# jantonguirao/nvImageCodec

Hardware: AMD Instinct MI355X
Metric: images/sec, batched 1920x1080 4:2:0 baseline JPEG decode to interleaved RGB u8 (higher is better)
Workload: dtype int32

## Files before the change

include/hipjpeg.h:

```cpp
#ifndef HIPJPEG_H_
#define HIPJPEG_H_

#include <stddef.h>
#include <stdint.h>

#ifdef __cplusplus
extern "C" {
#endif

#define HIPJPEG_API __attribute__((visibility("default")))

typedef enum {
    HIPJPEG_STATUS_SUCCESS = 0,
    HIPJPEG_STATUS_INVALID_ARGUMENT = 1,
    HIPJPEG_STATUS_BAD_JPEG = 2,
    HIPJPEG_STATUS_UNSUPPORTED = 3,
    HIPJPEG_STATUS_TRUNCATED = 4,
    HIPJPEG_STATUS_CORRUPT = 5,
    HIPJPEG_STATUS_ALLOC_FAILED = 6,
    HIPJPEG_STATUS_HIP_ERROR = 7,
    HIPJPEG_STATUS_NO_DEVICE = 8,
    HIPJPEG_STATUS_BUFFER_TOO_SMALL = 9,
    HIPJPEG_STATUS_INTERNAL_ERROR = 10
} hipjpegStatus_t;
// ... 44 lines not shown
    int32_t x0, y0, x1, y1;
    int32_t orientation;
} hipjpegTransform_t;

typedef struct hipjpegHandle* hipjpegHandle_t;

HIPJPEG_API const char* hipjpegStatusString(hipjpegStatus_t status);
HIPJPEG_API int hipjpegVersion(void);
HIPJPEG_API hipjpegStatus_t hipjpegTestSetFault(const char* site, int countdown);
HIPJPEG_API int hipjpegTestDoubleReports(void);
HIPJPEG_API int32_t hipjpegTestHostFallbacks(hipjpegHandle_t handle);
HIPJPEG_API hipjpegStatus_t hipjpegTestKernelFlavours(hipjpegHandle_t handle, int32_t plane_units[1], int32_t luma_units[3]);
HIPJPEG_API int32_t hipjpegTestFusedUnits(hipjpegHandle_t handle);

HIPJPEG_API int32_t hipjpegTestScanChunkDrops(const uint8_t* data, size_t length, int scan_index, uint32_t* drops, int32_t capacity);

HIPJPEG_API hipjpegStatus_t hipjpegGetImageInfo(const uint8_t* data, size_t length, hipjpegImageInfo_t* info);

HIPJPEG_API hipjpegStatus_t hipjpegEntropyDecodeHost(const uint8_t* data, size_t length, int16_t* coef, size_t coef_capacity_bytes,
                                                     uint64_t comp_offsets[4], uint16_t qtables[256]);

HIPJPEG_API hipjpegStatus_t hipjpegEntropyDecodeHostSparse(const uint8_t* data, size_t length, uint8_t* stream, size_t capacity_bytes, size_t* stream_bytes,
                                                           uint64_t table_offsets[4]);

HIPJPEG_API hipjpegStatus_t hipjpegEntropyDecodeGpuAlgorithmHost(const uint8_t* data, size_t length, int16_t* coef,
                                                                 size_t coef_capacity_bytes, uint64_t comp_offsets[4],
                                                                 int32_t* sync_passes);

HIPJPEG_API hipjpegStatus_t hipjpegCreate(hipjpegHandle_t* handle, int device_id, int num_host_threads);
HIPJPEG_API hipjpegStatus_t hipjpegDestroy(hipjpegHandle_t handle);
// ... 133 lines not shown
```

nvimagecodec_amd/_native.py:

```python
import ctypes
import os
import sys

_HERE = os.path.dirname(os.path.abspath(__file__))
LIB_PATH = os.environ.get("HIPJPEG_LIB_PATH") or os.path.join(_HERE, "libhipjpeg_ext.so")

STATUS_NAMES = {0: "SUCCESS", 1: "INVALID_ARGUMENT", 2: "BAD_JPEG", 3: "UNSUPPORTED", 4: "TRUNCATED", 5: "CORRUPT", 6: "ALLOC_FAILED",
                7: "HIP_ERROR", 8: "NO_DEVICE", 9: "BUFFER_TOO_SMALL", 10: "INTERNAL_ERROR"}

OUTPUT_RGBI, OUTPUT_BGRI, OUTPUT_RGB_PLANAR, OUTPUT_BGR_PLANAR, OUTPUT_Y, OUTPUT_YUV_PLANAR = range(6)
FLAG_FANCY_UPSAMPLING = 1
FLAG_GPU_HUFFMAN = 2
FLAG_GPU_RESTART_INTERVALS = 8
TRANSCODE_ORIENTATION_FROM_EXIF = 0x10000
TRANSCODE_TRIM = 0x20000
TRANSCODE_GRAYSCALE = 0x80000
TRANSCODE_CROP_EXPAND = 0x100000
TRANSCODE_COPY_MARKERS = 0x200000
FLAG_FAST_IDCT = 4


class HipJpegError(RuntimeError):
    def __init__(self, status, what=""):
        self.status = int(status)
# ... 89 lines not shown
    L.hipjpegDecodeBatchStats.argtypes = [vp, vp, vp, vp]
    L.hipjpegDecodeBatchGetStatuses.argtypes = [vp, vp, i32]
    L.hipjpegDecodeBatchSetTransforms.argtypes = [vp, vp, i32]
    L.hipjpegDecodeBatchSubmit.argtypes = [vp, vp, vp, i32, vp, i32, ctypes.c_uint, vp]
    L.hipjpegDecodeBatchWait.argtypes = [vp, vp, i32]
    L.hipjpegSetPipelineDepth.argtypes = [vp, i32]
    L.hipjpegSetHybridHuffmanThreshold.argtypes = [vp, ctypes.c_uint64]
    L.hipjpegDecodeBatchTransferStats.argtypes = [vp, ctypes.POINTER(ctypes.c_uint64), ctypes.POINTER(ctypes.c_int32)]
    L.hipjpegEntropyDecodeHostSparse.argtypes = [vp, sz, vp, sz, ctypes.POINTER(sz), vp]
    L.hipjpegDecodeBatchZeroCopyImages.argtypes = [vp]
    L.hipjpegDecodeBatchZeroCopyImages.restype = i32
    L.hipjpegTestHostFallbacks.argtypes = [vp]
    L.hipjpegTestHostFallbacks.restype = i32
    L.hipjpegTestScanChunkDrops.argtypes = [vp, ctypes.c_size_t, i32, ctypes.POINTER(ctypes.c_uint32), i32]
    L.hipjpegTestScanChunkDrops.restype = i32
    L.hipjpegTestKernelFlavours.argtypes = [vp, ctypes.POINTER(ctypes.c_int32), ctypes.POINTER(ctypes.c_int32)]
    L.hipjpegDecodeBatchEntropyStats.argtypes = [vp, ctypes.POINTER(ctypes.c_int32), ctypes.POINTER(ctypes.c_int32), ctypes.POINTER(ctypes.c_uint64)]
    L.hipjpegEncodeBatchDevice.argtypes = [vp, vp, vp, i32, vp, vp]
    L.hipjpegEncodeBatchRelaunch.argtypes = [vp, vp]
    L.hipjpegEncodeBatchHost.argtypes = [vp, vp]
    L.hipjpegEncodeBatchEntropy.argtypes = [vp, ctypes.c_uint, vp]
    L.hipjpegEncodeBatchSubmit.argtypes = [vp, vp, vp, i32, ctypes.c_uint, vp]
    L.hipjpegEncodeBatchWait.argtypes = [vp, vp, i32]
    L.hipjpegEncodeBatch.argtypes = [vp, vp, vp, i32, vp, vp]
    L.hipjpegEncodeGetBitstream.argtypes = [vp, i32, ctypes.POINTER(vp), ctypes.POINTER(sz)]
    L.hipjpegEncodeGetCoefficients.argtypes = [vp, i32, i32, ctypes.POINTER(vp), vp]
    L.hipjpegEncodeBatchStats.argtypes = [vp, vp, vp, vp]
    L.hipjpegEncodeBatchGpuEntropyImages.argtypes = [vp]
    L.hipjpegEncodeBatchGpuEntropyImages.restype = i32
    L.hipjpegEncodeFromCoefficientsHost.argtypes = [i32, i32, ctypes.POINTER(EncodeParams), vp, vp, sz, ctypes.POINTER(sz)]
# ... 21 lines not shown
```

nvimagecodec_amd/csrc/gpu_huffman.hip:

```cpp
#include <hip/hip_runtime.h>

#include "gpu_huffman.h"
#include "huffman_gpu_core.h"

namespace hipjpeg {

namespace {

constexpr int kThreads = 256;

constexpr int kRowShift = kSubseqWords == 32 ? 5 : kSubseqWords == 16 ? 4 : kSubseqWords == 64 ? 6 : -1;
static_assert(kRowShift > 0, "subsequences of 512, 1024 or 2048 bits");

#define HJ_LDS __attribute__((address_space(3)))
#define HJ_GLOBAL __attribute__((address_space(1)))
typedef unsigned int u32x4 __attribute__((ext_vector_type(4)));

struct KSlot {
    int16_t* base;
    uint32_t stride_y, stride_x;
};

constexpr int kStagedExtra = 2;
constexpr int kRowWords = kSubseqWords + kStagedExtra;
// ... 9 lines not shown
};

__device__ __forceinline__ uint32_t load_boundary(const uint32_t* boundaries, uint32_t n, uint32_t i)
{
    return i < n ? ((const HJ_GLOBAL uint32_t*)boundaries)[i] : 0xFFFFFFFFu;
}
#ifndef HJ_WALK_PARTS
#define HJ_WALK_PARTS 15
#endif
constexpr int kWalkParts = HJ_WALK_PARTS;
static_assert((kWalkParts & 4) == 0 || (kWalkParts & 3) == 3, "the select form needs the registers and the long step");
constexpr bool kLaneRegisters = (kWalkParts & 9) == 1, kLaneLongStep = (kWalkParts & 10) == 2;
typedef WalkPolicy<(kWalkParts & 2) != 0, (kWalkParts & 4) != 0> SyncWalk;
typedef WalkPolicy<kLaneLongStep, false> LaneWalk;

template <bool IN_VGPRS>
__device__ __forceinline__ TableClasses table_classes(const HuffImage& im)
{
    TableClasses c = make_table_classes(im.blocks_per_mcu, [&](uint32_t q) { return ((uint32_t)im.k[q].tdc * 2) | ((uint32_t)im.k[q].tac * 2 << 16); });
#pragma unroll
    for (int i = 0; i < 4; i++) {
        c.pair[i] = HJ_UNIFORM(c.pair[i]);
        if (IN_VGPRS) asm("" : "+v"(c.pair[i]));
    }
    c.bit0 = HJ_UNIFORM(c.bit0);
    c.bit1 = HJ_UNIFORM(c.bit1);
    return c;
}

struct DevEnv {
    uint32_t stream_base;
    uint32_t word0;
    uint32_t row_addr;
    uint32_t row_word0;
    uint32_t pool;
    const HJ_LDS uint32_t* tsel;
    TableClasses classes;
    const uint32_t* boundaries;
    uint32_t num_boundaries;
    __device__ __forceinline__ uint32_t boundary(uint32_t i) const { return load_boundary(boundaries, num_boundaries, i); }
    static constexpr uint32_t kCursorStep = (uint32_t)kSyncThreads * 4u;
    __device__ __forceinline__ void set_row(int row)
    {
        row_addr = stream_base + ((uint32_t)row << 2);
        row_word0 = word0 + ((uint32_t)row << kRowShift);
    }
    __device__ __forceinline__ uint32_t cursor(uint32_t i) const { return row_addr + (i - row_word0) * kCursorStep; }
    __device__ __forceinline__ uint32_t fetch(uint32_t c) const { return *(const HJ_LDS uint32_t*)(uintptr_t)c; }
    __device__ __forceinline__ uint32_t tables(int k) const { return kLaneRegisters ? select_tables(classes, (uint32_t)k) : tsel[k]; }
    __device__ __forceinline__ uint32_t lookup1(uint32_t t, uint32_t w) const
    {
        return *(const HJ_LDS uint16_t*)(uintptr_t)(pool + t + ((w >> (31 - kHuffFastBits)) & ((2u << kHuffFastBits) - 2)));
// ... 31 lines not shown
    return r;
}
__device__ __forceinline__ void put_mark(const SlotRecorder& r, uint32_t begin, uint32_t limit, uint32_t total_bits, uint32_t z0, const SubseqState& st)
{
    *(HJ_GLOBAL uint16_t*)(r.records + (r.off + 2 * kRecMark)) = (uint16_t)record_mark(begin, min(limit, total_bits), z0, st);
}

template <class Policy, class Env>
__device__ __forceinline__ SubseqState walk_with(bool rst, bool record, const HuffGeom& geom, const Env& env, uint32_t begin, uint32_t limit, int z, int k,
                                                 uint32_t boundary0, const SlotRecorder& rec)
{
    if (rst) return decode_subsequence<true, Env, NoRecord, Policy>(geom, env, begin, limit, z, k, boundary0);
    return record ? decode_subsequence<false, Env, SlotRecorder, Policy>(geom, env, begin, limit, z, k, 0, rec)
                  : decode_subsequence<false, Env, NoRecord, Policy>(geom, env, begin, limit, z, k);
}
template <class Env>
struct FourClasses : Env {
    __device__ __forceinline__ explicit FourClasses(const Env& e) : Env(e) {}
    __device__ __forceinline__ uint32_t tables(int k) const { return select_tables(this->classes, (uint32_t)k); }
};
template <class Env>
struct TwoClasses : Env {
    __device__ __forceinline__ explicit TwoClasses(const Env& e) : Env(e) {}
    __device__ __forceinline__ uint32_t tables(int k) const { return select_tables2(this->classes, (uint32_t)k); }
};
template <class Policy, class Env>
__device__ __forceinline__ SubseqState walk_subsequence(bool rst, bool record, const HuffGeom& geom, const Env& env, uint32_t begin, uint32_t limit, int z,
                                                        int k, uint32_t boundary0, const SlotRecorder& rec)
{
    if (Policy::kSelects) {
        if (env.classes.bit1 == 0) return walk_with<Policy>(rst, record, geom, TwoClasses<Env>(env), begin, limit, z, k, boundary0, rec);
        return walk_with<Policy>(rst, record, geom, FourClasses<Env>(env), begin, limit, z, k, boundary0, rec);
    }
    return walk_with<Policy>(rst, record, geom, env, begin, limit, z, k, boundary0, rec);
}

template <int ROWS>
__device__ __forceinline__ void stage_rows(uint32_t* lds_stream, const HuffImage& im, int first_row)
{
    const int t = threadIdx.x;
    const HJ_GLOBAL uint32_t* g = (const HJ_GLOBAL uint32_t*)im.stream;
    const int nwords = (int)im.stream_words;
    const int w0 = (first_row + t) * kSubseqWords;
    constexpr int kGroups = kSubseqWords / 4;
    u32x4 v[kGroups];
    typedef unsigned int u32x2 __attribute__((ext_vector_type(2)));
    u32x2 tail;
    {
        const int gd = w0 + kSubseqWords;
// ... 53 lines not shown
        constexpr uint8_t zz[64] = HJ_ZIGZAG_DEVICE_TABLE;
        const int i = (t - 64) * 4;
        zzw[t - 64] = ((uint32_t)zz[i] | ((uint32_t)zz[i + 1] << 8) | ((uint32_t)zz[i + 2] << 16) | ((uint32_t)zz[i + 3] << 24)) << 1;
    }
}

__device__ __forceinline__ DevEnv make_env(WgShared& sh, HJ_LDS uint16_t* pool, uint32_t first, const HuffGeom& geom, const HuffImage& im)
{
    DevEnv env;
    env.stream_base = (uint32_t)(uintptr_t)(HJ_LDS uint32_t*)sh.stream;
    env.word0 = (first - 1) * kSubseqWords;
    env.row_addr = env.stream_base;
    env.row_word0 = env.word0;
    env.pool = (uint32_t)(uintptr_t)pool;
    env.tsel = (const HJ_LDS uint32_t*)sh.tsel;
    env.classes = table_classes<true>(im);
    env.boundaries = geom.boundaries;
    env.num_boundaries = geom.num_boundaries;
    return env;
}

__device__ __forceinline__ int compact_tasks(WgShared& sh, bool has, int value, int* task)
{
    const int t = threadIdx.x;
    const unsigned long long mask = __ballot(has);
    const int below = __popcll(mask & ((1ull << (t & 63)) - 1));
    if ((t & 63) == 0) sh.wave_count[t >> 6] = (uint32_t)__popcll(mask);
    __syncthreads();
    int base = 0, n = 0;
#pragma unroll
    for (int w = 0; w < kSyncThreads / 64; w++) {
// ... 1304 lines not shown
```

nvimagecodec_amd/csrc/gpu_huffman_host.cpp:

```cpp
#include "gpu_huffman_host.h"

#include <algorithm>
#include <cstring>

namespace hipjpeg {

uint32_t scan_mcus_x(const FrameInfo& f, const ScanHeader& sc)
{
    return (uint32_t)(sc.ncomp == 1 ? (f.comp[sc.comp_index[0]].samp_w + 7) / 8 : f.mcus_x);
}

uint32_t scan_mcus_y(const FrameInfo& f, const ScanHeader& sc)
{
    return (uint32_t)(sc.ncomp == 1 ? (f.comp[sc.comp_index[0]].samp_h + 7) / 8 : f.mcus_y);
}

uint32_t scan_blocks_per_mcu(const FrameInfo& f, const ScanHeader& sc)
{
    if (sc.ncomp == 1) return 1;
    uint32_t n = 0;
    for (int i = 0; i < sc.ncomp; i++) n += (uint32_t)(f.comp[sc.comp_index[i]].h * f.comp[sc.comp_index[i]].v);
    return n;
}

// ... 109 lines not shown
        } else {
            const uint32_t prefix = code >> (l - kHuffFastBits);
            if ((first[prefix] >> 9) != kZadvLong) {
                first[prefix] = (uint16_t)(((base + used) / 64) | (kZadvLong << 9));
                for (int j = 0; j < (1 << kHuffSubBits); j++) pool[base + used + j] = (uint16_t)kEntryInvalid;
                used += 1u << kHuffSubBits;
            }
            uint16_t* sub = pool + (size_t)(first[prefix] & 0x1FFu) * 64;
            const uint32_t lo = (code & ((1u << (l - kHuffFastBits)) - 1)) << (16 - l);
            for (uint32_t j = 0; j < (1u << (16 - l)); j++) sub[lo + j] = e;
        }
    });
    if (!is_dc) {
        uint16_t* pair = first + kPairOffset;
        for (uint32_t w = 0; w < (1u << kHuffFastBits); w++) {
            pair[w] = 0;
            const uint32_t e1 = first[w], t1 = e1 & 31u, z1 = e1 >> 9;
            if (e1 == kEntryInvalid || z1 == kZadvLong || z1 == 64u || t1 + 2 > (uint32_t)kHuffFastBits) continue;
            const uint32_t e2 = first[(w << t1) & ((1u << kHuffFastBits) - 1)], t2 = e2 & 31u, z2 = e2 >> 9;
            if (e2 == kEntryInvalid || z2 == kZadvLong || t1 + t2 > (uint32_t)kHuffFastBits) continue;
            pair[w] = (uint16_t)make_pair_entry(t1 + t2, z2 == 64u ? 63u : z1 + z2, 64u - z1);
        }
    }
    return used;
}

}

size_t gpu_pool_words(const ScanHeader& sc)
{
    size_t words = 0;
    bool dc_seen[4] = {false, false, false, false}, ac_seen[4] = {false, false, false, false};
    for (int i = 0; i < sc.ncomp; i++) {
        const int td = sc.td[i], ta = sc.ta[i];
        if (!dc_seen[td]) {
            dc_seen[td] = true;
// ... 26 lines not shown
    }
    for (int i = 0; i < sc.ncomp; i++) {
        const int ta = sc.ta[i];
        if (!ac_seen[ta]) {
            ac_seen[ta] = true;
            ac_off[ta] = used;
            used += expand_table(sc.ac[ta], false, pool, used);
        }
    }
    im->pool_words = (uint32_t)used;
    for (uint32_t k = 0; k < im->blocks_per_mcu; k++) {
        const int c = im->k[k].comp;
        im->k[k].tdc = (uint16_t)dc_off[sc.td[c]];
        im->k[k].tac = (uint16_t)ac_off[sc.ta[c]];
    }
}

void fill_huff_image(const FrameInfo& f, const ScanHeader& sc, uint32_t stream_bytes, HuffImage* im)
{
    memset(im, 0, sizeof *im);
    im->total_bits = stream_bytes * 8u;
    im->num_subseq = (im->total_bits + kSubseqBits - 1) / kSubseqBits;
    im->stream_words = (uint32_t)((((size_t)stream_bytes + 3) & ~(size_t)3) + kStreamSlackBytes) / 4;
    im->mcus_x = scan_mcus_x(f, sc);
    im->mcus_y = scan_mcus_y(f, sc);
    im->ncomp = (uint32_t)sc.ncomp;
    int k = 0;
    for (int i = 0; i < sc.ncomp; i++) {
        const Component& fc = f.comp[sc.comp_index[i]];
        const int h = sc.ncomp == 1 ? 1 : fc.h, v = sc.ncomp == 1 ? 1 : fc.v;
// ... 31 lines not shown
    uint32_t second_table(uint32_t e) const { return (e & 0x1FFu) * 64u; }
    uint32_t lookup_pair(uint32_t t, uint32_t w) const
    {
        const size_t i = (size_t)t + kPairOffset + (w >> (32 - kHuffFastBits));
        return i < im->pool_words ? im->pool[i] : 0u;
    }
    uint32_t tables(int k) const { return (uint32_t)im->k[k].tdc | ((uint32_t)im->k[k].tac << 16); }
    int16_t* block_ptr(int k, uint32_t mx, uint32_t my) const
    {
        const HuffK& hk = im->k[k];
        return im->coef[hk.comp] + ((size_t)hk.blk0 + (size_t)my * hk.stride_y + (size_t)mx * hk.stride_x) * 64;
    }
    int zigzag(int z) const { return kZigzagDeviceGpuHost[z]; }
    int16_t* buf;
    void put(int index, int value) const { buf[index] = (int16_t)value; }
};

struct HostWindow {
    const HostEnv* env;
    uint32_t edc[64], eac[64];
    uint32_t tables(uint32_t k) const { return env->tables((int)k); }
    uint32_t entry(uint32_t table, uint32_t w) const
    {
        uint32_t e = env->lookup1(table, w);
        if ((e >> 9) == kZadvLong) e = env->lookup2(e, w);
        return e;
    }
    void open(uint32_t pos, uint32_t ts)
    {
        for (uint32_t l = 0; l < 64; l++) {
// ... 34 lines not shown
    im.pool = pool.data();
    im.dc_diff = dc_diff.data();
    im.boundaries = boundaries.data();
    im.num_boundaries = (uint32_t)boundaries.size();
    im.restart_interval = (uint32_t)sc.restart_interval;
    const bool rst = sc.restart_interval != 0;
    for (int i = 0; i < sc.ncomp; i++) {
        const int c = sc.comp_index[i];
        int16_t* const coef = frame_coef[c];
        im.coef[i] = coef;
        const size_t bw = (size_t)f.comp[c].blocks_w, rows = sc.ncomp == 1 ? im.mcus_y : (size_t)f.comp[c].blocks_h;
        const size_t cols = sc.ncomp == 1 ? im.mcus_x : bw;
        for (size_t y = 0; y < rows; y++) memset(coef + y * bw * 64, 0x5A, cols * 128);
    }
    int16_t block_buffer[64] = {0};
    const HostEnv env{&im, block_buffer};
    const HuffGeom geom = make_geom(im);
    const uint32_t ns = im.num_subseq;
    std::vector<SubseqState> cur(ns), nxt(ns);
    uint32_t err = 0;
    std::vector<uint16_t> records((size_t)ns * kRecShorts, 0);
    {
        const TableClasses classes = make_table_classes(im.blocks_per_mcu, [&](uint32_t q) { return env.tables((int)q); });
        if (!classes.complete) return 5;
        for (uint32_t q = 0; q < im.blocks_per_mcu; q++)
            if (select_tables(classes, q) != env.tables((int)q)) return 5;
    }
    bool policies_differ = false;
    uint16_t other[kRecShorts];
    auto walk = [&](uint32_t i, uint32_t begin, int z, int k, bool record) {
        const uint32_t limit = (i + 1) * kSubseqBits;
        uint16_t* rec = &records[(size_t)i * kRecShorts];
        if (rst) {
            rec[kRecMark] = (uint16_t)kRecInvalid;
            const SubseqState st = decode_subsequence<true, HostEnv, NoRecord, WalkSelects>(geom, env, begin, limit, z, k, 0);
            if (pack_state(st) != pack_state(decode_subsequence<true, HostEnv, NoRecord, WalkBranches>(geom, env, begin, limit, z, k, 0)) ||
                pack_state(st) != pack_state(decode_subsequence<true, HostEnv, NoRecord, WalkLongBranches>(geom, env, begin, limit, z, k, 0)))
                policies_differ = true;
            return st;
        }
        if (!record) {
// ... 136 lines not shown
```

nvimagecodec_amd/csrc/gpu_huffman_host.h:

```cpp
#pragma once
#include <cstddef>
#include <cstdint>
#include <vector>

#include "huffman_gpu_core.h"
#include "jpeg_syntax.h"

namespace hipjpeg {

constexpr int kMaxSeqScans = 4;
bool gpu_entropy_eligible(const FrameInfo& f);

uint32_t scan_mcus_x(const FrameInfo& f, const ScanHeader& sc);
uint32_t scan_mcus_y(const FrameInfo& f, const ScanHeader& sc);
uint32_t scan_blocks_per_mcu(const FrameInfo& f, const ScanHeader& sc);

inline size_t destuffed_capacity(const ScanHeader& sc) { return (((sc.data_end - sc.data_begin) + 3) & ~(size_t)3) + kStreamSlackBytes; }

size_t destuff_scan(const uint8_t* data, const ScanHeader& sc, uint8_t* out);

size_t gpu_pool_words(const ScanHeader& sc);

void build_gpu_pool(const ScanHeader& sc, HuffImage* im, uint16_t* pool);

void fill_huff_image(const FrameInfo& f, const ScanHeader& sc, uint32_t stream_bytes, HuffImage* im);

int emulate_gpu_entropy(const uint8_t* data, size_t size, const FrameInfo& f, int16_t* const coef[4], int* sync_passes);

}
```

nvimagecodec_amd/csrc/hipjpeg_api.cpp:

```cpp
#include <hip/hip_runtime_api.h>

#include <cstring>
#include <memory>
#include <new>
#include <vector>

#include "../../include/hipjpeg.h"
#include "coefficients_core.h"
#include "decoder_core.h"
#include "diagnostics.h"
#include "encoder_core.h"
#include "entropy_decode.h"
#include "gpu_huffman_encode.h"
#include "gpu_huffman_host.h"
#include "progressive_encode.h"
#include "progressive_gpu_host.h"
#include "thread_pool.h"
#include "transcode_core.h"

#include <chrono>
#include <future>
#include <cstdio>
#include <cstdlib>

// ... 463 lines not shown
int32_t hipjpegTestScanChunkDrops(const uint8_t* data, size_t length, int scan_index, uint32_t* drops, int32_t capacity)
{
    int32_t result = -1;
    if (!test_hooks_enabled()) return result;
    (void)guarded([&]() -> hipjpegStatus_t {
        hipjpeg::FrameInfo f;
        if (hipjpeg::parse_jpeg(data, length, &f) != hipjpeg::kParseOk || scan_index < 0 || scan_index >= (int)f.scans.size()) return HIPJPEG_STATUS_BAD_JPEG;
        const auto& d = f.scans[scan_index].chunk_drops;
        for (int32_t c = 0; c < (int32_t)d.size() && c < capacity && drops; c++) drops[c] = d[c];
        result = (int32_t)d.size();
        return HIPJPEG_STATUS_SUCCESS;
    });
    return result;
}

int32_t hipjpegTestHostFallbacks(hipjpegHandle_t handle)
{
    if (!handle || !test_hooks_enabled()) return -1;
    return handle->batches[handle->settled >= 0 ? handle->settled : handle->current]->host_fallback_images();
}

hipjpegStatus_t hipjpegTestKernelFlavours(hipjpegHandle_t handle, int32_t plane_units[1], int32_t luma_units[3])
{
    return guarded([&]() -> hipjpegStatus_t {
    if (!handle || !plane_units || !luma_units || !test_hooks_enabled()) return HIPJPEG_STATUS_INVALID_ARGUMENT;
    handle->cur().flavour_units(plane_units, luma_units);
    return HIPJPEG_STATUS_SUCCESS;
    });
}

// ... 422 lines not shown
```

nvimagecodec_amd/csrc/huffman_gpu_core.h:

```cpp
#pragma once
#include <cstdint>
#include <type_traits>

#if defined(__HIPCC__)
#include <hip/hip_runtime.h>
#define HJ_HD __host__ __device__ inline __attribute__((always_inline))
#else
#define HJ_HD inline
#endif

namespace hipjpeg {

#ifndef HJ_SUBSEQ_BITS
#define HJ_SUBSEQ_BITS 1024
#endif
#ifndef HJ_SYNC_THREADS
#define HJ_SYNC_THREADS 256
#endif
constexpr int kSubseqBits = HJ_SUBSEQ_BITS;
constexpr int kSubseqWords = kSubseqBits / 32;
constexpr int kHuffFastBits = 10;
constexpr int kHuffSubBits = 16 - kHuffFastBits;
constexpr int kStreamSlackBytes = 32;
constexpr int kSyncThreads = HJ_SYNC_THREADS;
constexpr int kHuffOwn = kSyncThreads - 1;
constexpr int kTailTaskBytes = 2 * kSyncThreads;
constexpr int kHuffBlocksPerWg = 256;
#ifndef HJ_MCUS_PER_WG
#define HJ_MCUS_PER_WG 128
#endif
constexpr int kHuffMcusPerWg = HJ_MCUS_PER_WG;
constexpr int kDestuffChunk = 16384;
constexpr int kMaxPoolWords = 12288;

HJ_HD constexpr uint32_t make_entry(uint32_t total, uint32_t nb, uint32_t zadv) { return total | (nb << 5) | (zadv << 9); }
constexpr uint32_t kPairOffset = 1u << kHuffFastBits;
HJ_HD constexpr uint32_t make_pair_entry(uint32_t total, uint32_t zadv, uint32_t z_below) { return total | (zadv << 4) | (z_below << 10); }
constexpr uint32_t kEntryInvalid = 1u | (15u << 5) | (1u << 9);
constexpr uint32_t kZadvLong = 127;

struct HuffK {
    uint32_t blk0;
    uint32_t stride_y;
    uint16_t tdc, tac;
    uint8_t comp;
    uint8_t stride_x;
    uint8_t pad[2];
};

struct alignas(16) HuffImage {
    const uint8_t* stream;
    const uint16_t* pool;
    int16_t* coef[4];
    int16_t* dc_diff;
// ... 200 lines not shown
HJ_HD uint32_t bit_select(uint32_t mask, uint32_t ones, uint32_t zeros) { return (mask & ones) | (~mask & zeros); }
HJ_HD uint32_t bit_mask(uint32_t bits, uint32_t k)
{
#if defined(__HIP_DEVICE_COMPILE__)
    return (uint32_t)__builtin_amdgcn_sbfe((int)bits, k, 1u);
#else
    return 0u - ((bits >> k) & 1u);
#endif
}
HJ_HD uint32_t select_tables(const TableClasses& c, uint32_t k)
{
    const uint32_t a = bit_mask(c.bit0, k), b = bit_mask(c.bit1, k);
    return bit_select(b, bit_select(a, c.pair[3], c.pair[2]), bit_select(a, c.pair[1], c.pair[0]));
}
HJ_HD uint32_t select_tables2(const TableClasses& c, uint32_t k) { return bit_select(bit_mask(c.bit0, k), c.pair[1], c.pair[0]); }

template <bool LONG_STEP, bool SELECTS>
struct WalkPolicy {
    static constexpr bool kLongStep = LONG_STEP, kSelects = SELECTS;
    static_assert(LONG_STEP || !SELECTS, "the select form has no memory read to predicate");
};
typedef WalkPolicy<false, false> WalkBranches;
typedef WalkPolicy<true, false> WalkLongBranches;
typedef WalkPolicy<true, true> WalkSelects;
HJ_HD uint32_t sub_window(uint32_t w) { return (w << kHuffFastBits) >> (kHuffFastBits - kHuffSubBits); }

template <bool RST, class Env, class Rec = NoRecord, class Policy = WalkBranches>
HJ_HD SubseqState decode_subsequence(const HuffGeom& im, const Env& env, uint32_t begin, uint32_t limit, int z, int k, uint32_t boundary0 = 0,
                                     Rec rec = Rec())
{
    static_assert(!RST || std::is_same<Rec, NoRecord>::value, "records are not taken across restart boundaries");
    uint32_t pos = begin, nblocks = 0;
    const uint32_t end = limit < im.total_bits ? limit : im.total_bits;
    const uint32_t pair_end = end > (uint32_t)kHuffFastBits - 2 ? end - ((uint32_t)kHuffFastBits - 2) : 0;
    const int bpm = (int)im.blocks_per_mcu;
    uint32_t tsel = env.tables(k);
    uint32_t tcur = z == 0 ? (tsel & 0xFFFFu) : (tsel >> 16);
    BitReader br;
    br.start(env, pos);
    RestartCursor rc;
    if (RST) {
        rc.start(env, boundary0, pos);
        if (rc.normalise(env, br.hi, &pos, &z, &k)) {
            tsel = env.tables(k);
            tcur = tsel & 0xFFFFu;
            br.start(env, pos);
        }
    }
    const uint32_t fresh = z == 0 ? 1u : 0u;
    if (fresh && pos < end) rec(0u, pos);
    uint32_t win = br.hi;
    bool sub = false;
    while (pos < end) {
        const uint32_t fetched = env.fetch(br.next);
        uint32_t e = env.lookup1(tcur, win);
        const uint32_t pr = env.lookup_pair(tcur, win);
        const bool two = z != 0 && (uint32_t)z < (pr >> 10) && pos < pair_end && !sub;
        uint32_t tot = two ? (pr & 15u) : (e & 31u);
        bool mcu_done = false;
        if (Policy::kSelects) {
            const uint32_t zadv1 = e >> 9, zadv2 = (pr >> 4) & 63u, t2 = env.second_table(e);
            const bool lng = !two & (zadv1 == kZadvLong) & !sub;
            tot = lng ? 0u : tot;
            uint32_t zadv = two ? zadv2 : zadv1;
            zadv = lng ? 0u : zadv;
            z += (int)zadv;
            const bool done = z >= 64;
            if (done) rec(nblocks + fresh, pos + tot);
            z = done ? 0 : z;
            nblocks += done ? 1u : 0u;
            int k1 = k + 1;
            k1 = k1 == bpm ? 0 : k1;
            k = done ? k1 : k;
            tsel = env.tables(k);
            const uint32_t tdc = tsel & 0xFFFFu, tac = tsel >> 16;
            tcur = lng ? t2 : tac;
            tcur = done ? tdc : tcur;
            mcu_done = done & (k == 0);
            sub = lng;
        } else if (Policy::kLongStep) {
            const bool was_sub = sub;
            sub = false;
            tcur = tsel >> 16;
            z += two ? (int)((pr >> 4) & 63u) : (int)(e >> 9);
            if (z >= 64) {
                if (!two && (e >> 9) == kZadvLong && !was_sub) {
                    z -= (int)kZadvLong;
                    tot = 0;
                    tcur = env.second_table(e);
                    sub = true;
                } else {
                    z = 0;
                    rec(nblocks + fresh, pos + tot);
                    nblocks++;
                    if (++k == bpm) k = 0;
                    tsel = env.tables(k);
                    tcur = tsel & 0xFFFFu;
                    mcu_done = k == 0;
                }
            }
        } else {
            tcur = tsel >> 16;
            z += two ? (int)((pr >> 4) & 63u) : (int)(e >> 9);
            if (z >= 64) {
                if (!two && (e >> 9) == kZadvLong) {
                    e = env.lookup2(e, br.hi);
                    z += (int)(e >> 9) - (int)kZadvLong;
                    tot = e & 31u;
                }
                if (z >= 64) {
                    z = 0;
                    rec(nblocks + fresh, pos + tot);
                    nblocks++;
                    if (++k == bpm) k = 0;
                    tsel = env.tables(k);
                    tcur = tsel & 0xFFFFu;
                    mcu_done = k == 0;
                }
            }
        }
        pos += tot;
        br.consume(tot, fetched);
        if (RST && mcu_done && rc.normalise(env, br.hi, &pos, &z, &k)) {
            tsel = env.tables(k);
            tcur = tsel & 0xFFFFu;
            br.start(env, pos);
        }
        const uint32_t behind = sub_window(br.hi);
        win = sub ? behind : br.hi;
    }
    SubseqState st;
    st.end_bit = pos;
    st.zk = (uint16_t)((k << 8) | z);
    st.nblocks = (uint16_t)(nblocks > 0xFFFF ? 0xFFFF : nblocks);
    return st;
}

#if defined(__HIP_DEVICE_COMPILE__)
#define HJ_UNIFORM(x) ((uint32_t)__builtin_amdgcn_readfirstlane((int)(x)))
#else
#define HJ_UNIFORM(x) ((uint32_t)(x))
#endif
template <class Win>
HJ_HD uint32_t cooperative_table_changes(const Win& win, uint32_t blocks_per_mcu)
// ... 70 lines not shown
        rc.start(env, boundary0, pos);
        const uint32_t met = rc.index;
        if (rc.normalise(env, br.hi, &pos, &z, &k, fault)) {
            tsel = env.tables(k);
            tcur = tsel & 0xFFFFu;
            br.start(env, pos);
            fresh = true;
        }
        if (fault && rc.index != met && block != (met + 1) * im.interval_blocks) *fault = 1;
    }
    if (fresh && pos < end) rec(block, pos);
    while (pos < end) {
        const uint32_t fetched = env.fetch(br.next);
        uint32_t e = env.lookup1(tcur, br.hi);
        const uint32_t pr = env.lookup_pair(tcur, br.hi);
        const bool two = z != 0 && (uint32_t)z < (pr >> 10) && pos < pair_end;
        if (!two && (e >> 9) == kZadvLong) e = env.lookup2(e, br.hi);
        const uint32_t tot = two ? (pr & 15u) : (e & 31u);
        pos += tot;
        br.consume(tot, fetched);
        z += two ? (int)((pr >> 4) & 63u) : (int)(e >> 9);
        tcur = tsel >> 16;
        if (z >= 64) {
            z = 0;
            block++;
            if (++k == bpm) k = 0;
            tsel = env.tables(k);
            tcur = tsel & 0xFFFFu;
            if (RST && k == 0) {
                const uint32_t met = rc.index;
                if (rc.normalise(env, br.hi, &pos, &z, &k, fault)) {
                    tsel = env.tables(k);
                    tcur = tsel & 0xFFFFu;
                    br.start(env, pos);
                }
                if (fault && rc.index != met && block != (met + 1) * im.interval_blocks) *fault = 1;
// ... 70 lines not shown
```

Before: 108,400.

## Unify pair-table entry format and add countdown table-select walk for GPU Huffman

Pair-table entries now use the same encoding as single-code entries, with the fallback entry stored when no pair fits. The pair-eligibility test moves to a branch-free comparison on the first entry, so the walk no longer needs the z_below field. A new select_walk path counts MCU blocks down and keeps per-class DC/AC table pointers split and pinned in VGPRs. This is meant to cut per-symbol selection and bit-extraction ALU work in the selects policy. It also adds a test hook and host emulation checks, at the cost of more live registers.

```diff
diff --git a/include/hipjpeg.h b/include/hipjpeg.h
--- a/include/hipjpeg.h
+++ b/include/hipjpeg.h
@@ -82,6 +82,7 @@
 HIPJPEG_API int32_t hipjpegTestFusedUnits(hipjpegHandle_t handle);
 
 HIPJPEG_API int32_t hipjpegTestScanChunkDrops(const uint8_t* data, size_t length, int scan_index, uint32_t* drops, int32_t capacity);
+HIPJPEG_API int32_t hipjpegTestPairSteps(const uint8_t bits[16], const uint8_t* vals, int32_t nvals, uint32_t* steps);
 
 HIPJPEG_API hipjpegStatus_t hipjpegGetImageInfo(const uint8_t* data, size_t length, hipjpegImageInfo_t* info);
 
diff --git a/nvimagecodec_amd/_native.py b/nvimagecodec_amd/_native.py
--- a/nvimagecodec_amd/_native.py
+++ b/nvimagecodec_amd/_native.py
@@ -127,6 +127,8 @@
     L.hipjpegTestHostFallbacks.restype = i32
     L.hipjpegTestScanChunkDrops.argtypes = [vp, ctypes.c_size_t, i32, ctypes.POINTER(ctypes.c_uint32), i32]
     L.hipjpegTestScanChunkDrops.restype = i32
+    L.hipjpegTestPairSteps.argtypes = [vp, vp, i32, vp]
+    L.hipjpegTestPairSteps.restype = i32
     L.hipjpegTestKernelFlavours.argtypes = [vp, ctypes.POINTER(ctypes.c_int32), ctypes.POINTER(ctypes.c_int32)]
     L.hipjpegDecodeBatchEntropyStats.argtypes = [vp, ctypes.POINTER(ctypes.c_int32), ctypes.POINTER(ctypes.c_int32), ctypes.POINTER(ctypes.c_uint64)]
     L.hipjpegEncodeBatchDevice.argtypes = [vp, vp, vp, i32, vp, vp]
diff --git a/nvimagecodec_amd/csrc/gpu_huffman.hip b/nvimagecodec_amd/csrc/gpu_huffman.hip
--- a/nvimagecodec_amd/csrc/gpu_huffman.hip
+++ b/nvimagecodec_amd/csrc/gpu_huffman.hip
@@ -47,10 +47,11 @@
 typedef WalkPolicy<(kWalkParts & 2) != 0, (kWalkParts & 4) != 0> SyncWalk;
 typedef WalkPolicy<kLaneLongStep, false> LaneWalk;
 
-template <bool IN_VGPRS>
+template <bool IN_VGPRS, bool COUNTDOWN = false>
 __device__ __forceinline__ TableClasses table_classes(const HuffImage& im)
 {
-    TableClasses c = make_table_classes(im.blocks_per_mcu, [&](uint32_t q) { return ((uint32_t)im.k[q].tdc * 2) | ((uint32_t)im.k[q].tac * 2 << 16); });
+    const auto of = [&](uint32_t q) { return ((uint32_t)im.k[q].tdc * 2) | ((uint32_t)im.k[q].tac * 2 << 16); };
+    TableClasses c = COUNTDOWN ? make_countdown_classes(im.blocks_per_mcu, of) : make_table_classes(im.blocks_per_mcu, of);
 #pragma unroll
     for (int i = 0; i < 4; i++) {
         c.pair[i] = HJ_UNIFORM(c.pair[i]);
@@ -69,6 +70,7 @@
     uint32_t pool;
     const HJ_LDS uint32_t* tsel;
     TableClasses classes;
+    StepTables step;
     const uint32_t* boundaries;
     uint32_t num_boundaries;
     __device__ __forceinline__ uint32_t boundary(uint32_t i) const { return load_boundary(boundaries, num_boundaries, i); }
@@ -130,25 +132,30 @@
     return record ? decode_subsequence<false, Env, SlotRecorder, Policy>(geom, env, begin, limit, z, k, 0, rec)
                   : decode_subsequence<false, Env, NoRecord, Policy>(geom, env, begin, limit, z, k);
 }
-template <class Env>
-struct FourClasses : Env {
-    __device__ __forceinline__ explicit FourClasses(const Env& e) : Env(e) {}
-    __device__ __forceinline__ uint32_t tables(int k) const { return select_tables(this->classes, (uint32_t)k); }
-};
-template <class Env>
-struct TwoClasses : Env {
-    __device__ __forceinline__ explicit TwoClasses(const Env& e) : Env(e) {}
-    __device__ __forceinline__ uint32_t tables(int k) const { return select_tables2(this->classes, (uint32_t)k); }
+template <class Env, bool FOUR>
+struct StepEnv : Env {
+    __device__ __forceinline__ explicit StepEnv(const Env& e) : Env(e) {}
+    __device__ __forceinline__ void step_tables(uint32_t d, uint32_t* tdc, uint32_t* tac) const { select_halves<FOUR>(this->step, d, tdc, tac); }
+    __device__ __forceinline__ uint32_t step_entry(uint32_t t, uint32_t w) const
+    {
+        return *(const HJ_LDS uint16_t*)(uintptr_t)(t + ((w >> (31 - kHuffFastBits)) & ((2u << kHuffFastBits) - 2)));
+    }
+    __device__ __forceinline__ uint32_t step_pair(uint32_t t, uint32_t w) const
+    {
+        return *(const HJ_LDS uint16_t*)(uintptr_t)(t + 2 * kPairOffset + ((w >> (31 - kHuffFastBits)) & ((2u << kHuffFastBits) - 2)));
+    }
+    __device__ __forceinline__ uint32_t step_second(uint32_t e) const { return second_table_of(e, 7u, this->pool); }
 };
 template <class Policy, class Env>
 __device__ __forceinline__ SubseqState walk_subsequence(bool rst, bool record, const HuffGeom& geom, const Env& env, uint32_t begin, uint32_t limit, int z,
                                                         int k, uint32_t boundary0, const SlotRecorder& rec)
 {
-    if (Policy::kSelects) {
-        if (env.classes.bit1 == 0) return walk_with<Policy>(rst, record, geom, TwoClasses<Env>(env), begin, limit, z, k, boundary0, rec);
-        return walk_with<Policy>(rst, record, geom, FourClasses<Env>(env), begin, limit, z, k, boundary0, rec);
-    }
-    return walk_with<Policy>(rst, record, geom, env, begin, limit, z, k, boundary0, rec);
+    if constexpr (Policy::kSelects) {
+        if (env.classes.bit1 == 0) return walk_with<Policy>(rst, record, geom, StepEnv<Env, false>(env), begin, limit, z, k, boundary0, rec);
+        return walk_with<Policy>(rst, record, geom, StepEnv<Env, true>(env), begin, limit, z, k, boundary0, rec);
+    } else {
+        return walk_with<Policy>(rst, record, geom, env, begin, limit, z, k, boundary0, rec);
+    }
 }
 
 template <int ROWS>
@@ -232,7 +239,14 @@
     env.row_word0 = env.word0;
     env.pool = (uint32_t)(uintptr_t)pool;
     env.tsel = (const HJ_LDS uint32_t*)sh.tsel;
-    env.classes = table_classes<true>(im);
+    const TableClasses down = table_classes<true, true>(im);
+    env.classes = kLaneRegisters ? table_classes<true>(im) : down;
+    env.step = split_classes(down, 1u, env.pool);
+#pragma unroll
+    for (int i = 0; i < 4; i++) {
+        asm("" : "+v"(env.step.dc[i]));
+        asm("" : "+v"(env.step.ac[i]));
+    }
     env.boundaries = geom.boundaries;
     env.num_boundaries = geom.num_boundaries;
     return env;
diff --git a/nvimagecodec_amd/csrc/gpu_huffman_host.cpp b/nvimagecodec_amd/csrc/gpu_huffman_host.cpp
--- a/nvimagecodec_amd/csrc/gpu_huffman_host.cpp
+++ b/nvimagecodec_amd/csrc/gpu_huffman_host.cpp
@@ -147,12 +147,12 @@
     if (!is_dc) {
         uint16_t* pair = first + kPairOffset;
         for (uint32_t w = 0; w < (1u << kHuffFastBits); w++) {
-            pair[w] = 0;
             const uint32_t e1 = first[w], t1 = e1 & 31u, z1 = e1 >> 9;
+            pair[w] = (uint16_t)e1;
             if (e1 == kEntryInvalid || z1 == kZadvLong || z1 == 64u || t1 + 2 > (uint32_t)kHuffFastBits) continue;
             const uint32_t e2 = first[(w << t1) & ((1u << kHuffFastBits) - 1)], t2 = e2 & 31u, z2 = e2 >> 9;
             if (e2 == kEntryInvalid || z2 == kZadvLong || t1 + t2 > (uint32_t)kHuffFastBits) continue;
-            pair[w] = (uint16_t)make_pair_entry(t1 + t2, z2 == 64u ? 63u : z1 + z2, 64u - z1);
+            pair[w] = (uint16_t)make_pair_entry(t1 + t2, z2 == 64u ? 63u : z1 + z2);
         }
     }
     return used;
@@ -209,6 +209,22 @@
         im->k[k].tdc = (uint16_t)dc_off[sc.td[c]];
         im->k[k].tac = (uint16_t)ac_off[sc.ta[c]];
     }
+}
+
+bool pair_table_steps(const HuffSpec& ac, uint32_t* out)
+{
+    const size_t words = table_words(ac, false);
+    if (!words || words > (size_t)kMaxPoolWords) return false;
+    std::vector<uint16_t> pool(words);
+    expand_table(ac, false, pool.data(), 0);
+    for (uint32_t w = 0; w < (1u << kHuffFastBits); w++)
+        for (uint32_t z = 0; z < 64; z++) {
+            const uint32_t e = pool[w], pr = pool[kPairOffset + w];
+            const bool two = pair_fits(z, e), lng = e >= (kZadvLong << 9);
+            const uint32_t x = lng ? 0u : two ? pr : e;
+            out[w * 64 + z] = (x & 31u) | ((x >> 9) << 8) | ((two && pr != e ? 1u : 0u) << 16) | ((lng ? 1u : 0u) << 17);
+        }
+    return true;
 }
 
 void fill_huff_image(const FrameInfo& f, const ScanHeader& sc, uint32_t stream_bytes, HuffImage* im)
@@ -270,6 +286,15 @@
     int zigzag(int z) const { return kZigzagDeviceGpuHost[z]; }
     int16_t* buf;
     void put(int index, int value) const { buf[index] = (int16_t)value; }
+    TableClasses classes;
+    StepTables step;
+    void step_tables(uint32_t d, uint32_t* tdc, uint32_t* tac) const
+    {
+        select_halves<true>(step, d, tdc, tac);
+    }
+    uint32_t step_entry(uint32_t t, uint32_t w) const { return lookup1(t, w); }
+    uint32_t step_pair(uint32_t t, uint32_t w) const { return lookup_pair(t, w); }
+    uint32_t step_second(uint32_t e) const { return second_table_of(e, 6u, 0u); }
 };
 
 struct HostWindow {
@@ -334,7 +359,9 @@
         for (size_t y = 0; y < rows; y++) memset(coef + y * bw * 64, 0x5A, cols * 128);
     }
     int16_t block_buffer[64] = {0};
-    const HostEnv env{&im, block_buffer};
+    HostEnv env{&im, block_buffer, TableClasses(), StepTables()};
+    env.classes = make_countdown_classes(im.blocks_per_mcu, [&](uint32_t q) { return env.tables((int)q); });
+    env.step = split_classes(env.classes, 1u, 0u);
     const HuffGeom geom = make_geom(im);
     const uint32_t ns = im.num_subseq;
     std::vector<SubseqState> cur(ns), nxt(ns);
@@ -345,6 +372,12 @@
         if (!classes.complete) return 5;
         for (uint32_t q = 0; q < im.blocks_per_mcu; q++)
             if (select_tables(classes, q) != env.tables((int)q)) return 5;
+        if (!env.classes.complete) return 5;
+        for (uint32_t q = 0; q < im.blocks_per_mcu; q++) {
+            uint32_t tdc, tac;
+            env.step_tables(im.blocks_per_mcu - 1u - q, &tdc, &tac);
+            if ((tdc | (tac << 16)) != env.tables((int)q)) return 5;
+        }
     }
     bool policies_differ = false;
     uint16_t other[kRecShorts];
diff --git a/nvimagecodec_amd/csrc/gpu_huffman_host.h b/nvimagecodec_amd/csrc/gpu_huffman_host.h
--- a/nvimagecodec_amd/csrc/gpu_huffman_host.h
+++ b/nvimagecodec_amd/csrc/gpu_huffman_host.h
@@ -23,6 +23,8 @@
 
 void build_gpu_pool(const ScanHeader& sc, HuffImage* im, uint16_t* pool);
 
+bool pair_table_steps(const HuffSpec& ac, uint32_t* out);
+
 void fill_huff_image(const FrameInfo& f, const ScanHeader& sc, uint32_t stream_bytes, HuffImage* im);
 
 int emulate_gpu_entropy(const uint8_t* data, size_t size, const FrameInfo& f, int16_t* const coef[4], int* sync_passes);
diff --git a/nvimagecodec_amd/csrc/hipjpeg_api.cpp b/nvimagecodec_amd/csrc/hipjpeg_api.cpp
--- a/nvimagecodec_amd/csrc/hipjpeg_api.cpp
+++ b/nvimagecodec_amd/csrc/hipjpeg_api.cpp
@@ -501,6 +501,21 @@
     return result;
 }
 
+int32_t hipjpegTestPairSteps(const uint8_t bits[16], const uint8_t* vals, int32_t nvals, uint32_t* steps)
+{
+    int32_t result = -1;
+    if (!test_hooks_enabled() || !bits || !vals || !steps || nvals < 0 || nvals > 256) return result;
+    (void)guarded([&]() -> hipjpegStatus_t {
+        hipjpeg::HuffSpec spec;
+        for (int l = 1; l <= 16; l++) spec.bits[l] = bits[l - 1];
+        for (int32_t i = 0; i < nvals; i++) spec.vals[i] = vals[i];
+        spec.present = true;
+        if (hipjpeg::pair_table_steps(spec, steps)) result = 0;
+        return HIPJPEG_STATUS_SUCCESS;
+    });
+    return result;
+}
+
 int32_t hipjpegTestHostFallbacks(hipjpegHandle_t handle)
 {
     if (!handle || !test_hooks_enabled()) return -1;
diff --git a/nvimagecodec_amd/csrc/huffman_gpu_core.h b/nvimagecodec_amd/csrc/huffman_gpu_core.h
--- a/nvimagecodec_amd/csrc/huffman_gpu_core.h
+++ b/nvimagecodec_amd/csrc/huffman_gpu_core.h
@@ -35,9 +35,10 @@
 
 HJ_HD constexpr uint32_t make_entry(uint32_t total, uint32_t nb, uint32_t zadv) { return total | (nb << 5) | (zadv << 9); }
 constexpr uint32_t kPairOffset = 1u << kHuffFastBits;
-HJ_HD constexpr uint32_t make_pair_entry(uint32_t total, uint32_t zadv, uint32_t z_below) { return total | (zadv << 4) | (z_below << 10); }
+constexpr uint32_t kZadvLong = 127;
+HJ_HD constexpr uint32_t make_pair_entry(uint32_t total, uint32_t zadv) { return make_entry(total, 0u, zadv); }
+HJ_HD bool pair_fits(uint32_t z, uint32_t e) { return (z << 9) - 512u < 0x7E00u - e; }
 constexpr uint32_t kEntryInvalid = 1u | (15u << 5) | (1u << 9);
-constexpr uint32_t kZadvLong = 127;
 
 struct HuffK {
     uint32_t blk0;
@@ -268,6 +269,40 @@
     return bit_select(b, bit_select(a, c.pair[3], c.pair[2]), bit_select(a, c.pair[1], c.pair[0]));
 }
 HJ_HD uint32_t select_tables2(const TableClasses& c, uint32_t k) { return bit_select(bit_mask(c.bit0, k), c.pair[1], c.pair[0]); }
+struct StepTables {
+    uint32_t dc[4], ac[4];
+    uint32_t bit0, bit1;
+};
+template <class TablesOf>
+HJ_HD TableClasses make_countdown_classes(uint32_t blocks_per_mcu, const TablesOf& of)
+{
+    return make_table_classes(blocks_per_mcu, [&](uint32_t q) { return of(blocks_per_mcu - 1u - q); });
+}
+HJ_HD StepTables split_classes(const TableClasses& c, uint32_t unit, uint32_t base)
+{
+    StepTables s;
+    for (int i = 0; i < 4; i++) {
+        s.dc[i] = base + (c.pair[i] & 0xFFFFu) * unit;
+        s.ac[i] = base + (c.pair[i] >> 16) * unit;
+    }
+    s.bit0 = c.bit0;
+    s.bit1 = c.bit1;
+    return s;
+}
+template <bool FOUR>
+HJ_HD void select_halves(const StepTables& s, uint32_t d, uint32_t* tdc, uint32_t* tac)
+{
+    const uint32_t a = bit_mask(s.bit0, d);
+    if (FOUR) {
+        const uint32_t b = bit_mask(s.bit1, d);
+        *tdc = bit_select(b, bit_select(a, s.dc[3], s.dc[2]), bit_select(a, s.dc[1], s.dc[0]));
+        *tac = bit_select(b, bit_select(a, s.ac[3], s.ac[2]), bit_select(a, s.ac[1], s.ac[0]));
+    } else {
+        *tdc = bit_select(a, s.dc[1], s.dc[0]);
+        *tac = bit_select(a, s.ac[1], s.ac[0]);
+    }
+}
+HJ_HD uint32_t second_table_of(uint32_t e, uint32_t shift, uint32_t base) { return (e << shift) + (base - (kZadvLong << (9u + shift))); }
 
 template <bool LONG_STEP, bool SELECTS>
 struct WalkPolicy {
@@ -279,11 +314,85 @@
 typedef WalkPolicy<true, true> WalkSelects;
 HJ_HD uint32_t sub_window(uint32_t w) { return (w << kHuffFastBits) >> (kHuffFastBits - kHuffSubBits); }
 
+template <bool RST, class Env, class Rec>
+HJ_HD SubseqState select_walk(const HuffGeom& im, const Env& env, uint32_t begin, uint32_t limit, int z0, int k0, uint32_t boundary0, Rec rec)
+{
+    uint32_t pos = begin, nblocks = 0, z = (uint32_t)z0;
+    const uint32_t end = limit < im.total_bits ? limit : im.total_bits;
+    const uint32_t pair_end = end > (uint32_t)kHuffFastBits - 2 ? end - ((uint32_t)kHuffFastBits - 2) : 0;
+    const uint32_t bpm1 = im.blocks_per_mcu - 1u;
+    uint32_t d = bpm1 - (uint32_t)k0;
+    uint32_t tdc, tac;
+    env.step_tables(d, &tdc, &tac);
+    uint32_t tcur = z == 0 ? tdc : tac;
+    BitReader br;
+    br.start(env, pos);
+    RestartCursor rc;
+    if (RST) {
+        rc.start(env, boundary0, pos);
+        int zi = (int)z, ki = k0;
+        if (rc.normalise(env, br.hi, &pos, &zi, &ki)) {
+            z = (uint32_t)zi;
+            d = bpm1 - (uint32_t)ki;
+            env.step_tables(d, &tdc, &tac);
+            tcur = tdc;
+            br.start(env, pos);
+        }
+    }
+    const uint32_t fresh = z == 0 ? 1u : 0u;
+    if (fresh && pos < end) rec(0u, pos);
+    uint32_t win = br.hi;
+    bool sub = false;
+    while (pos < end) {
+        const uint32_t fetched = env.fetch(br.next);
+        const uint32_t e = env.step_entry(tcur, win);
+        const uint32_t pr = env.step_pair(tcur, win);
+        const bool two = pair_fits(z, e) & (pos < pair_end) & !sub;
+        const bool lng = (e >= (kZadvLong << 9)) & !sub;
+        uint32_t x = two ? pr : e;
+        x = lng ? 0u : x;
+        const uint32_t tot = x & 31u, zadv = x >> 9;
+        const uint32_t t2 = env.step_second(e);
+        z += zadv;
+        const bool done = z >= 64u;
+        if (done) rec(nblocks + fresh, pos + tot);
+        z = done ? 0u : z;
+        nblocks += done ? 1u : 0u;
+        d -= done ? 1u : 0u;
+        d = d < bpm1 ? d : bpm1;
+        const bool mcu_done = done & (d == bpm1);
+        env.step_tables(d, &tdc, &tac);
+        tcur = lng ? t2 : tac;
+        tcur = done ? tdc : tcur;
+        sub = lng;
+        pos += tot;
+        br.consume(tot, fetched);
+        if (RST && mcu_done) {
+            int zi = (int)z, ki = 0;
+            if (rc.normalise(env, br.hi, &pos, &zi, &ki)) {
+                z = (uint32_t)zi;
+                d = bpm1;
+                env.step_tables(d, &tdc, &tac);
+                tcur = tdc;
+                br.start(env, pos);
+            }
+        }
+        const uint32_t behind = sub_window(br.hi);
+        win = sub ? behind : br.hi;
+    }
+    SubseqState st;
+    st.end_bit = pos;
+    st.zk = (uint16_t)(((bpm1 - d) << 8) | z);
+    st.nblocks = (uint16_t)(nblocks > 0xFFFF ? 0xFFFF : nblocks);
+    return st;
+}
+
 template <bool RST, class Env, class Rec = NoRecord, class Policy = WalkBranches>
 HJ_HD SubseqState decode_subsequence(const HuffGeom& im, const Env& env, uint32_t begin, uint32_t limit, int z, int k, uint32_t boundary0 = 0,
                                      Rec rec = Rec())
 {
     static_assert(!RST || std::is_same<Rec, NoRecord>::value, "records are not taken across restart boundaries");
+    if constexpr (Policy::kSelects) return select_walk<RST>(im, env, begin, limit, z, k, boundary0, rec);
     uint32_t pos = begin, nblocks = 0;
     const uint32_t end = limit < im.total_bits ? limit : im.total_bits;
     const uint32_t pair_end = end > (uint32_t)kHuffFastBits - 2 ? end - ((uint32_t)kHuffFastBits - 2) : 0;
@@ -307,41 +416,22 @@
     bool sub = false;
     while (pos < end) {
         const uint32_t fetched = env.fetch(br.next);
-        uint32_t e = env.lookup1(tcur, win);
+        const uint32_t e = env.lookup1(tcur, win);
         const uint32_t pr = env.lookup_pair(tcur, win);
-        const bool two = z != 0 && (uint32_t)z < (pr >> 10) && pos < pair_end && !sub;
-        uint32_t tot = two ? (pr & 15u) : (e & 31u);
+        const bool two = pair_fits((uint32_t)z, e) && pos < pair_end && !sub;
+        const uint32_t x = two ? pr : e;
+        uint32_t tot = x & 31u;
         bool mcu_done = false;
-        if (Policy::kSelects) {
-            const uint32_t zadv1 = e >> 9, zadv2 = (pr >> 4) & 63u, t2 = env.second_table(e);
-            const bool lng = !two & (zadv1 == kZadvLong) & !sub;
-            tot = lng ? 0u : tot;
-            uint32_t zadv = two ? zadv2 : zadv1;
-            zadv = lng ? 0u : zadv;
-            z += (int)zadv;
-            const bool done = z >= 64;
-            if (done) rec(nblocks + fresh, pos + tot);
-            z = done ? 0 : z;
-            nblocks += done ? 1u : 0u;
-            int k1 = k + 1;
-            k1 = k1 == bpm ? 0 : k1;
-            k = done ? k1 : k;
-            tsel = env.tables(k);
-            const uint32_t tdc = tsel & 0xFFFFu, tac = tsel >> 16;
-            tcur = lng ? t2 : tac;
-            tcur = done ? tdc : tcur;
-            mcu_done = done & (k == 0);
-            sub = lng;
-        } else if (Policy::kLongStep) {
+        tcur = tsel >> 16;
+        z += (int)(x >> 9);
+        if (Policy::kLongStep) {
             const bool was_sub = sub;
             sub = false;
-            tcur = tsel >> 16;
-            z += two ? (int)((pr >> 4) & 63u) : (int)(e >> 9);
             if (z >= 64) {
-                if (!two && (e >> 9) == kZadvLong && !was_sub) {
+                if ((x >> 9) == kZadvLong && !was_sub) {
                     z -= (int)kZadvLong;
                     tot = 0;
-                    tcur = env.second_table(e);
+                    tcur = env.second_table(x);
                     sub = true;
                 } else {
                     z = 0;
@@ -354,13 +444,11 @@
                 }
             }
         } else {
-            tcur = tsel >> 16;
-            z += two ? (int)((pr >> 4) & 63u) : (int)(e >> 9);
             if (z >= 64) {
-                if (!two && (e >> 9) == kZadvLong) {
-                    e = env.lookup2(e, br.hi);
-                    z += (int)(e >> 9) - (int)kZadvLong;
-                    tot = e & 31u;
+                if ((x >> 9) == kZadvLong) {
+                    const uint32_t e2 = env.lookup2(x, br.hi);
+                    z += (int)(e2 >> 9) - (int)kZadvLong;
+                    tot = e2 & 31u;
                 }
                 if (z >= 64) {
                     z = 0;
@@ -380,8 +468,12 @@
             tcur = tsel & 0xFFFFu;
             br.start(env, pos);
         }
-        const uint32_t behind = sub_window(br.hi);
-        win = sub ? behind : br.hi;
+        if (Policy::kLongStep) {
+            const uint32_t behind = sub_window(br.hi);
+            win = sub ? behind : br.hi;
+        } else {
+            win = br.hi;
+        }
     }
     SubseqState st;
     st.end_bit = pos;
@@ -482,12 +574,13 @@
         const uint32_t fetched = env.fetch(br.next);
         uint32_t e = env.lookup1(tcur, br.hi);
         const uint32_t pr = env.lookup_pair(tcur, br.hi);
-        const bool two = z != 0 && (uint32_t)z < (pr >> 10) && pos < pair_end;
-        if (!two && (e >> 9) == kZadvLong) e = env.lookup2(e, br.hi);
-        const uint32_t tot = two ? (pr & 15u) : (e & 31u);
+        const bool two = pair_fits((uint32_t)z, e) && pos < pair_end;
+        e = two ? pr : e;
+        if ((e >> 9) == kZadvLong) e = env.lookup2(e, br.hi);
+        const uint32_t tot = e & 31u;
         pos += tot;
         br.consume(tot, fetched);
-        z += two ? (int)((pr >> 4) & 63u) : (int)(e >> 9);
+        z += (int)(e >> 9);
         tcur = tsel >> 16;
         if (z >= 64) {
             z = 0;
```

Measured after the change: 112,900, median of 6. +4.1%, better.
